# sd-james/gym-treasure-game

Hardware: AMD Instinct MI355X
Metric: env-steps/sec (whole node) at 1M batched envs, 1/2/4/8 MI355X; bit-exact vs CPU (higher is better)
Workload: dtype int32+f64

## Files before the change

gym-treasure-game_amd/csrc/tg_core.h:

```cpp
#pragma once
#include <hip/hip_runtime.h>
#include <stdint.h>

#define TG_HD __host__ __device__ __forceinline__

namespace tg {

constexpr int S = 48;
constexpr int INCR = S / 10;
constexpr int HALFW = S / 4;
constexpr int MT_N = 624, MT_M = 397;
constexpr int TICK_CAP = 1 << 14;
constexpr uint32_t TICK_DRAWS = 8;
constexpr uint32_t MAX_TICK_DRAWS = 48;
constexpr int PAD = 2;

enum : uint32_t { B_OPEN = 1, B_LADDER = 2, B_WALL = 4, B_DOOR = 8, B_DOOROBJ = 16  };
enum : int { P_NOP = 0, P_UP, P_DOWN, P_LEFT, P_RIGHT, P_JUMP, P_INTERACT };
enum : int { O_GO_LEFT = 0, O_GO_RIGHT, O_UP_LADDER, O_DOWN_LADDER, O_INTERACT, O_DOWN_LEFT,
             O_DOWN_RIGHT, O_JUMP_LEFT, O_JUMP_RIGHT, O_COUNT };

constexpr uint32_t F_JT = 0x1Fu;
constexpr uint32_t F_FACING = 1u << 5;
constexpr int F_OBJ = 6;
// ... 133 lines not shown
};
__host__ __device__ inline __attribute__((noinline)) WordPair mt_pair_ool(const uint32_t* mt, uint32_t p) {
  WordPair r;
  mt_pair(mt, p, r.w0, r.w1);
  return r;
}
TG_HD uint32_t mt_half(uint32_t pos) { return pos >= (uint32_t)MT_HALF ? (uint32_t)MT_HALF : 0u; }

constexpr int MT_CODES = MT_WORDS / 2;
constexpr uint32_t CODE_POS = 3u;
constexpr uint32_t CODE_NEG_SHIFT = 2;
constexpr uint32_t CODE_JUMP = 1u << 4;
constexpr uint32_t CODE_FLIP = 1u << 5;
TG_HD uint32_t draw_code(double r) {
  const uint32_t pos = (uint32_t)((int)rint(2.0 + 2.0 * r) - 2);
  const uint32_t neg = (uint32_t)((int)rint(-4.0 + 2.0 * r) + 4);
  return pos | (neg << CODE_NEG_SHIFT) | (r > 0.25 ? CODE_JUMP : 0u) | (r <= 0.8 ? CODE_FLIP : 0u);
}
constexpr uint32_t CODE_SLOW = 0xFFu;
TG_HD uint32_t code_of_top27(uint32_t a) {
  constexpr uint32_t Q1 = 1u << 25, Q3 = 3u << 25, F8 = 107374182u;
  if (a - (Q1 - 1u) < 3u || a - (Q3 - 1u) < 3u || a - (F8 - 1u) < 3u) return CODE_SLOW;
  constexpr uint32_t LOW = CODE_FLIP;
  constexpr uint32_t MID = 1u | (1u << CODE_NEG_SHIFT) | CODE_JUMP | CODE_FLIP;
  constexpr uint32_t HIGH = 2u | (2u << CODE_NEG_SHIFT) | CODE_JUMP;
  return a < Q1 ? LOW : a < Q3 ? MID : a < F8 ? (HIGH | CODE_FLIP) : HIGH;
}
TG_HD uint32_t draw_code_words(uint32_t w0, uint32_t w1) {
  const uint32_t c = code_of_top27(mt_temper(w0) >> 5);
  return c != CODE_SLOW ? c : draw_code(mt_double(w0, w1));
}
constexpr uint32_t TOP27_F8 = 107374182u;
constexpr uint32_t TOP27_LUT = CODE_FLIP |
                               ((1u | (1u << CODE_NEG_SHIFT) | CODE_JUMP | CODE_FLIP) << 8) |
                               ((1u | (1u << CODE_NEG_SHIFT) | CODE_JUMP | CODE_FLIP) << 16) |
                               ((2u | (2u << CODE_NEG_SHIFT) | CODE_JUMP | CODE_FLIP) << 24);
static_assert(TOP27_F8 >= (3u << 25), "only the top class splits at 0.8");
TG_HD bool top27_slow(uint32_t a) {
  return (((a + 1u) & 0x1FFFFFFu) < 3u) | (a - (TOP27_F8 - 1u) < 3u);
}
TG_HD uint32_t top27_code(uint32_t a) {
  const uint32_t c = (TOP27_LUT >> ((a >> 22) & 0x18u)) & 0xFFu;
  return a >= TOP27_F8 ? c ^ CODE_FLIP : c;
}
TG_HD int code_step(uint32_t c, bool neg) {
  return neg ? (int)((c >> CODE_NEG_SHIFT) & 3u) - 4 : (int)(c & CODE_POS) + 2;
}
TG_HD void gen_codes(const uint32_t* words, uint8_t* c) {
  for (int k = 0; k < MT_N / 2; ++k) c[k] = (uint8_t)draw_code(mt_double(words[2 * k], words[2 * k + 1]));
}
struct GenOps {
  TG_HD void twist(const uint32_t* src, uint32_t* dst) const { twist_gen(src, dst); }
  TG_HD void codes(const uint32_t* w, uint8_t* c) const { gen_codes(w, c); }
};
template <class Ops = GenOps>
TG_HD void twist_half(uint32_t* mt, uint32_t h, uint8_t* mc = nullptr, bool seeded = false,
                      const Ops& op = Ops()) {
  const uint32_t g0 = h / (uint32_t)MT_N;
  uint32_t* const s = mt + mt_store_off(g0);
  uint32_t* const s3 = s + 3 * MT_N;
  if (!seeded) op.twist(mt + mt_store_off((g0 + (uint32_t)MT_HALF_GENS + 6u) % (2u * MT_HALF_GENS)), s3);
  uint8_t* const c = mc ? mc + h / 2 : nullptr;
  const int last = c ? MT_HALF_GENS : MT_HALF_GENS - 1;
  for (int g = 0; g < last; ++g) {
    const int to = (g + 1) >> 1 < 3 ? (g + 1) >> 1 : 3;
    const uint32_t* const from = g == 0 ? s3 : (g & 1) ? s + (g >> 1) * MT_N : s + to * MT_N;
    op.twist(from, s + to * MT_N);
    if (c) op.codes(s + to * MT_N, c + g * (MT_N / 2));
  }
  if (c) {
    op.twist(s + 2 * MT_N, s3);
    op.twist(s3, s3);
  }
}

template <int DIR, class R>
TG_HD int walk_ticks(R& rng, int& x, int lim, int cap) {
  int t = 0;
  while ((DIR > 0 ? x <= lim : x >= lim) && rng.has(TICK_DRAWS) && t < cap) {
    x += code_step(rng.code(), DIR < 0);
    ++t;
  }
  return t;
}

struct Rng {
  uint32_t* mt;
  uint32_t pos;
  uint32_t draws;
  bool crossed;
  bool entered;
  uint8_t* mc;

  TG_HD Rng(uint32_t* m, uint32_t state, uint8_t* c = nullptr)
      : mt(m), pos(state & MT_POS_MASK), draws(0u), crossed((state & MT_STALE) != 0u),
        entered(false), mc(c) {}

  TG_HD double random() {
    uint32_t w0, w1;
    mt_pair_branchy(mt, pos, w0, w1);
    pos += 2;
    if (pos == (uint32_t)MT_WORDS) pos = 0u;
    if (pos == 0u || pos == (uint32_t)MT_HALF) {
      if (crossed) twist_half(mt, pos, mc);
      crossed = entered = true;
    }
    ++draws;
    return mt_double(w0, w1);
  }
  TG_HD double uniform(double a, double b) { return a + (b - a) * random(); }
  TG_HD uint32_t code() { return draw_code(random()); }
  TG_HD void reserve(uint32_t) {}
  TG_HD bool has(uint32_t) const { return true; }
  TG_HD bool overrun() const { return false; }
  TG_HD void phase(int) {}
  template <int DIR>
  TG_HD int walk(int& x, int lim, int cap) { return walk_ticks<DIR>(*this, x, lim, cap); }
  TG_HD uint32_t finish() const { return pos | (crossed ? MT_STALE : 0u); }
  TG_HD uint32_t finish_queued() const { return pos | (entered ? MT_STALE : 0u); }
};
TG_HD uint32_t refill_after(uint32_t* mt, uint32_t state, uint8_t* mc = nullptr) {
  const uint32_t pos = state & MT_POS_MASK;
  if (state & MT_STALE) twist_half(mt, (uint32_t)MT_HALF - mt_half(pos), mc);
  return pos;
}

TG_HD void seed_mt(uint32_t* mt, const uint32_t* genrand19650218, uint64_t seed) {
  const uint32_t key0 = (uint32_t)seed, key1 = (uint32_t)(seed >> 32);
  const uint32_t klen = key1 ? 2u : 1u;
  uint32_t prev = genrand19650218[0];
  uint32_t m0 = prev;
  uint32_t j = 0;
  uint32_t i = 1;
  for (int k = 0; k < MT_N; ++k) {
    const uint32_t cur = (i == 1 && k == MT_N - 1) ? mt[1] : genrand19650218[i];
    const uint32_t key = (j == 0) ? key0 : key1;
    const uint32_t v = (cur ^ ((prev ^ (prev >> 30)) * 1664525u)) + key + j;
    mt[i] = v;
    prev = v;
    ++i;
    ++j;
    if (i >= (uint32_t)MT_N) { m0 = mt[MT_N - 1]; prev = m0; i = 1; }
    if (j >= klen) j = 0;
  }
  mt[0] = m0;
  for (int k = 0; k < MT_N - 1; ++k) {
    const uint32_t cur = mt[i];
    const uint32_t v = (cur ^ ((prev ^ (prev >> 30)) * 1566083941u)) - i;
    mt[i] = v;
    prev = v;
    ++i;
    if (i >= (uint32_t)MT_N) { mt[0] = mt[MT_N - 1]; prev = mt[0]; i = 1; }
  }
  mt[0] = 0x80000000u;
}
constexpr uint32_t MT_SEED_OFF = 3 * MT_N;
TG_HD void init_mt(uint32_t* mt, const uint32_t* genrand19650218, uint64_t seed,
                   uint8_t* mc = nullptr) {
  seed_mt(mt + MT_SEED_OFF, genrand19650218, seed);
  twist_half(mt, 0u, mc, true);
  twist_half(mt, (uint32_t)MT_HALF, mc);
}

struct AirCells {
  uint32_t oA, oB, bA, bB;
  int bx, by1;
// ... 703 lines not shown
    if (!pr.lad(DIR, y) || pr.fall(dc, y)) break;
    int end;
    if (DIR < 0) {
      end = max(max(floordiv(y - INCR, S) * S + INCR, floordiv(y, S) * S),
                max(floordiv(y + S - INCR, S) * S - (S - INCR), floordiv(y + S + 2, S) * S - (S + 2)));
      end = max(end, bound);
    } else {
      end = min(min(floordiv(y, S) * S + S - 1, floordiv(y + S / 2, S) * S + S - 1 - S / 2),
                min(floordiv(y + S + INCR - 1, S) * S + S - 1 - (S + INCR - 1),
                    floordiv(y + S + 2, S) * S + S - 1 - (S + 2)));
      end = min(end, bound);
    }
    lim = end;
    y = end + DIR;
  }
  return lim;
}

template <int K, class R>
TG_HD int air_tick(const Level& L, const uint32_t* trig, const Map& m, Env& e, Opt& o, R& rng,
                   AirCells& ac) {
  constexpr int DIR = (K == O_JUMP_LEFT || K == O_DOWN_LEFT) ? -1 : 1;
  constexpr bool JUMP = K == O_JUMP_LEFT || K == O_JUMP_RIGHT;
  const uint32_t dc = Map::dc_of(e.f);
  if (!ac.holds(dc, e.px, e.py)) {
    ac = m.air_cells(dc, e.px, e.py);
    if (!ac.holds(dc, e.px, e.py)) {
      const int prim = policy<K>(L, m, e, o);
      return tick<prims_of(K), R>(L, trig, m, e, prim, rng);
    }
  }
  const AirProbe ap(ac, e.px, e.py);
  const bool cf0 = ap.can_fall();
  const bool fwd = ap.side(DIR);
  int mv = 0;
  if (close_x(e, o.tx)) {
    if (!cf0) o.done = true;
  } else {
    mv = (JUMP && !cf0 && !fwd) ? -DIR : DIR;
  }
  int xd = 0, yd = 0;
  if (mv != 0 && (mv == DIR ? fwd : ap.side(-DIR))) {
    xd = code_step(rng.code(), mv < 0);
    e.f = mv > 0 ? (e.f | F_FACING) : (e.f & ~F_FACING);
  }
  const uint32_t jt = e.f & F_JT;
  if (jt > 0) {
    if (ap.up_clear()) yd = -INCR;
    e.f = (e.f & ~F_JT) | (jt - 1);
  } else if (cf0) {
    yd = INCR;
  }
  e.px += xd;
  if (yd > 0) yd = ap.fall(e.px, yd);
  e.py += yd;
  pickups(L, e);
  return -1;
}

template <int DIR, class R>
TG_HD int ladder_tick(const Level& L, const Map& m, const LadMasks& lm, Env& e, Opt& o, R& rng) {
  int yd = 0;
  if (DIR < 0 ? lm.can_go_up(m, e.py) : lm.can_go_down(m, e.py)) yd = code_step(rng.code(), DIR < 0);
  else o.done = true;
  const uint32_t jt = e.f & F_JT;
  if (jt > 0) {
    if (lm.up_clear(m, e.py)) yd = -INCR;
    e.f = (e.f & ~F_JT) | (jt - 1);
  } else if (lm.can_fall(m, e.py)) {
    yd = INCR;
  }
  if (yd > 0) yd = lm.fall_dist(m, e.py, yd);
  e.py += yd;
  pickups(L, e);
  return -1;
}

template <int DIR, class R, class P, class Full>
TG_HD void ladder_loop(const Level& L, const Map& m, Env& e, Opt& o, R& rng, StepResult& r,
                       const P& pr, Full full) {
  int lim = DIR > 0 ? -0x40000000 : 0x40000000;
  do {
    rng.phase(0);
    bool capped = false;
    while ((DIR > 0 ? e.py <= lim : e.py >= lim) && rng.has(TICK_DRAWS)) {
      e.py += code_step(rng.code(), DIR < 0);
      r.reward += -1;
      if (DIR > 0 ? e.py > lim : e.py < lim) pickups(L, e);
      if (++r.ticks >= TICK_CAP) {
        e.f |= E_TICKCAP;
        capped = true;
        lim = DIR > 0 ? -0x40000000 : 0x40000000;
      }
    }
    if (capped) break;
    rng.phase(1);
    rng.reserve(TICK_DRAWS);
    rng.phase(2);
    r.reward += full();
    if (!o.done) lim = ladder_plain_limit<DIR>(m, e, pr);
    rng.phase(3);
    if (++r.ticks >= TICK_CAP) {
      e.f |= E_TICKCAP;
      break;
    }
  } while (!o.done);
}

template <int K, class R>
TG_HD void run_option_k(const Level& L, const uint32_t* trig, const Map& m, Env& e, R& rng,
                        StepResult& r) {
  r.ran = 1;
  Opt o{0, false, false};
  if constexpr (K == O_GO_LEFT || K == O_GO_RIGHT) {
    constexpr int DIR = K == O_GO_LEFT ? -1 : 1;
    int lim = DIR > 0 ? -0x40000000 : 0x40000000;
    do {
      rng.phase(0);
      if (const int t = rng.template walk<DIR>(e.px, lim, TICK_CAP - r.ticks)) {
        e.f = DIR > 0 ? (e.f | F_FACING) : (e.f & ~F_FACING);
        r.reward -= t;
        r.ticks += t;
        if (DIR > 0 ? e.px > lim : e.px < lim) pickups(L, e);
        if (r.ticks >= TICK_CAP) {
          e.f |= E_TICKCAP;
          break;
        }
      }
      rng.phase(1);
      rng.reserve(TICK_DRAWS);
      rng.phase(2);
      const int prim = policy<K>(L, m, e, o);
      r.reward += tick<prims_of(K), R>(L, trig, m, e, prim, rng);
      if (!o.done) lim = go_plain_limit<DIR>(m, e, o.tx);
      rng.phase(3);
      if (++r.ticks >= TICK_CAP) {
        e.f |= E_TICKCAP;
        break;
      }
    } while (!o.done);
    return;
  }
  if constexpr (K == O_UP_LADDER || K == O_DOWN_LADDER) {
    constexpr int DIR = K == O_UP_LADDER ? -1 : 1;
    if (m.mk) {
      const LadMasks lm(m, Map::dc_of(e.f), e.px);
      ladder_loop<DIR>(L, m, e, o, rng, r, LadProbeMk{m, lm},
                       [&]() { return ladder_tick<DIR>(L, m, lm, e, o, rng); });
      return;
    }
    ladder_loop<DIR>(L, m, e, o, rng, r, LadProbe{m, e}, [&]() {
      const int prim = policy<K>(L, m, e, o);
      return tick<prims_of(K), R>(L, trig, m, e, prim, rng);
    });
    return;
  }
  if constexpr (K == O_JUMP_LEFT || K == O_JUMP_RIGHT || K == O_DOWN_LEFT || K == O_DOWN_RIGHT) {
    AirCells ac{0u, 0u, 0u, 0u, -0x40000000, 0, 0u};
    do {
      rng.phase(0);
      rng.phase(1);
      rng.reserve(TICK_DRAWS);
      rng.phase(2);
      if (o.init) {
        r.reward += air_tick<K>(L, trig, m, e, o, rng, ac);
      } else {
        const int prim = policy<K>(L, m, e, o);
        r.reward += tick<prims_of(K), R>(L, trig, m, e, prim, rng);
      }
      rng.phase(3);
      if (++r.ticks >= TICK_CAP) {
        e.f |= E_TICKCAP;
        break;
      }
    } while (!o.done);
    return;
  }
  do {
    rng.reserve(K == O_INTERACT ? L.interact_draws : TICK_DRAWS);
    const int prim = policy<K>(L, m, e, o);
    r.reward += tick<prims_of(K), R>(L, trig, m, e, prim, rng);
    if (++r.ticks >= TICK_CAP) {
      e.f |= E_TICKCAP;
      break;
    }
  } while (!o.done);
}
template <class R>
TG_HD void run_option(const Level& L, const uint32_t* trig, const Map& m, Env& e, int k,
                      R& rng, StepResult& r) {
  switch (k) {
    case O_GO_LEFT: run_option_k<O_GO_LEFT>(L, trig, m, e, rng, r); break;
    case O_GO_RIGHT: run_option_k<O_GO_RIGHT>(L, trig, m, e, rng, r); break;
    case O_UP_LADDER: run_option_k<O_UP_LADDER>(L, trig, m, e, rng, r); break;
    case O_DOWN_LADDER: run_option_k<O_DOWN_LADDER>(L, trig, m, e, rng, r); break;
    case O_INTERACT: run_option_k<O_INTERACT>(L, trig, m, e, rng, r); break;
    case O_DOWN_LEFT: run_option_k<O_DOWN_LEFT>(L, trig, m, e, rng, r); break;
    case O_DOWN_RIGHT: run_option_k<O_DOWN_RIGHT>(L, trig, m, e, rng, r); break;
    case O_JUMP_LEFT: run_option_k<O_JUMP_LEFT>(L, trig, m, e, rng, r); break;
    default: run_option_k<O_JUMP_RIGHT>(L, trig, m, e, rng, r); break;
  }
}
TG_HD int option_index(int a) {
  if (a < -O_COUNT || a >= O_COUNT) return -1;
  return a < 0 ? a + O_COUNT : a;
}
template <class R>
TG_HD StepResult env_step(const Level& L, const uint32_t* trig, const Map& m, Env& e, int a,
                          R& rng) {
  StepResult r{0, 0, 0, 0};
  const int k = option_index(a);
  if (k < 0) e.f |= E_ACTION;
  else if (can_run(L, m, e, k)) run_option(L, trig, m, e, k, rng, r);
  r.done = is_done(e);
  return r;
}

}
```

gym-treasure-game_amd/csrc/tg_dev.h:

```cpp
#pragma once
#include <hip/hip_runtime.h>

#include "../../include/tg_amd.h"
#include "tg_core.h"
#include "tg_level.h"
#include "tg_batch.h"
#include "tg_twist.h"

using namespace tg;

namespace {

constexpr int BLOCK = 256;
#ifndef TG_RUN_BLOCK
#define TG_RUN_BLOCK 256
#endif
constexpr int RUN_BLOCK = TG_RUN_BLOCK;
static_assert(RUN_BLOCK % 64 == 0 && BLOCK % RUN_BLOCK == 0, "whole waves, whole k_classify blocks");
constexpr int PRIO_SLOW = 3;

__device__ __forceinline__ void unpack_st4(const uint4 s, Env& e) {
  e.px = (int)(int16_t)(s.x & 0xFFFFu);
  e.py = (int)(int16_t)(s.x >> 16);
  e.f = s.y;
// ... 119 lines not shown
__device__ __noinline__ WordPair mt_pair_ool_sc1(const uint32_t* mt, uint32_t p) {
  WordPair r;
  mt_pair(mt, p, r.w0, r.w1, Sc1Ld());
  return r;
}

template <bool FLOW = false>
struct RngCodesT {
  static constexpr uint32_t NONE = 0xFFFFFFFFu;
  uint32_t* mt;
  uint8_t* mc;
  lds_u8* cell;
  uint32_t m0;
  uint32_t pos;
  uint32_t n;
  uint32_t rd;
  uint32_t left;
  uint32_t nxc;
  uint32_t stale;
  uint32_t tag;
  uint32_t draws;
  uint32_t regens;
  bool primed, loaded, entered;

  __device__ __forceinline__ RngCodesT(uint32_t* m, uint8_t* c, uint32_t state, lds_u8* wave_win)
      : mt(m), mc(c), cell(wave_win + (threadIdx.x & 63) * WIN_UNIT),
        m0(__builtin_amdgcn_readfirstlane((uint32_t)(uintptr_t)wave_win)),
        pos(state & MT_POS_MASK), n(0u), rd(0u), left(0u), nxc(0u),
        stale((state & MT_STALE) ? (uint32_t)MT_HALF - mt_half(state & MT_POS_MASK) : NONE),
        tag(state & (MT_STALE | MT_LISTED)),
        draws(0u), regens(0u), primed(false), loaded(false), entered(false) {}

  __device__ __forceinline__ void sync() {
    const uint32_t d = pos >> 1, e = d + n;
    if (e / (MT_HALF / 2) != d / (MT_HALF / 2)) {
      const uint32_t left_half = mt_half(pos), entered_half = (uint32_t)MT_HALF - left_half;
      if (stale == entered_half) {
        if (FLOW) regen_half_flow(mt, mc, entered_half);
        else regen_half(mt, mc, entered_half);
        ++regens;
      }
      stale = left_half;
      entered = true;
    }
    pos = 2u * (e >= (uint32_t)MT_CODES ? e - (uint32_t)MT_CODES : e);
    n = 0u;
  }
  __device__ __forceinline__ void fill() {
    const uint32_t d = pos >> 1, c0 = d / (uint32_t)WIN_UNIT;
    if (stale != NONE) {
      const uint32_t w0 = pos, w1 = pos + 2u * ((uint32_t)WIN_DRAWS - d % (uint32_t)WIN_UNIT);
      if ((w0 < stale + (uint32_t)MT_HALF && stale < w1) ||
          (w1 > (uint32_t)MT_WORDS && stale < w1 - (uint32_t)MT_WORDS)) {
        if (FLOW) regen_half_flow(mt, mc, stale);
        else regen_half(mt, mc, stale);
        ++regens;
        stale = NONE;
      }
    }
#pragma unroll
    for (int j = 0; j < WIN_SLOTS; ++j) {
      const uint32_t c = c0 + j < CODE_UNITS ? c0 + j : c0 + j - CODE_UNITS;
      glds_unit<FLOW>(m0 + j * WIN_SLOT_BYTES, mc + c * (uint32_t)WIN_UNIT);
    }
    rd = d % (uint32_t)WIN_UNIT;
    left = (uint32_t)WIN_DRAWS - rd;
    loaded = false;
  }
  __device__ __forceinline__ uint32_t read() const {
    const uint32_t r = rd < (uint32_t)WIN_DRAWS ? rd : 0u;
    return cell[(r / WIN_UNIT) * WIN_SLOT_BYTES + r % WIN_UNIT];
  }
  __device__ __forceinline__ void prime() {
    fill();
    primed = true;
  }
  __device__ __forceinline__ void reserve(uint32_t k) {
    if (!primed) prime();
    if (left < k) {
      asm volatile("s_waitcnt lgkmcnt(0)" ::: "memory");
      sync();
      fill();
    }
    if (!loaded) {
      asm volatile("s_waitcnt vmcnt(0)" ::: "memory");
      nxc = read();
      loaded = true;
    }
  }
  __device__ __forceinline__ bool has(uint32_t k) const { return left >= k; }
  __device__ __forceinline__ uint32_t dword(uint32_t d) const {
    return *reinterpret_cast<const lds_u32*>(cell + (4u * d / WIN_UNIT) * WIN_SLOT_BYTES +
                                             (4u * d) % WIN_UNIT);
  }
  template <int DIR>
  __device__ __forceinline__ int walk(int& x, const int lim, const int cap) {
    int taken = 0;
    if (!((DIR > 0 ? x <= lim : x >= lim) && left >= TICK_DRAWS && cap > 0)) return 0;
    uint32_t w = dword(rd >> 2);
    while (true) {
      const uint32_t wn = dword((rd >> 2) + 1u);
      const int k = (int)(rd & 3u);
      int moved = 0;
      bool act = true;
#pragma unroll
      for (int i = 0; i < 4; ++i) {
        const int st = code_step((w >> (8 * i)) & 0xFFu, DIR < 0);
        act = act && (i >= k ? ((DIR > 0 ? x <= lim : x >= lim) &&
                                left - (uint32_t)moved >= TICK_DRAWS && taken + moved < cap)
                             : true);
        if (i >= k && act) {
          x += st;
          ++moved;
        }
      }
      taken += moved;
      rd += (uint32_t)moved;
      left -= (uint32_t)moved;
      n += (uint32_t)moved;
      draws += (uint32_t)moved;
      if (moved < 4 - k) break;
      if (!((DIR > 0 ? x <= lim : x >= lim) && left >= TICK_DRAWS && taken < cap)) break;
      w = wn;
    }
    nxc = read();
    return taken;
  }
#ifdef TG_DIAG_STAMPS
  unsigned long long ph[4] = {0, 0, 0, 0}, last = 0;
  uint32_t rounds = 0;
  __device__ __forceinline__ void phase(int k) {
    const unsigned long long now = __builtin_amdgcn_s_memtime();
    if (last) ph[k] += now - last;
    last = now;
    rounds += k == 0;
  }
#else
  __device__ __forceinline__ void phase(int) {}
#endif
  __device__ __forceinline__ bool overrun() const { return left > (uint32_t)WIN_DRAWS; }
  __device__ __forceinline__ uint32_t code() {
    const uint32_t c = nxc;
    ++n;
    ++draws;
    ++rd;
    --left;
    nxc = read();
    return c;
  }
  __device__ __forceinline__ double random() {
    uint32_t p = (pos >> 1) + n;
    p = 2u * (p >= (uint32_t)MT_CODES ? p - (uint32_t)MT_CODES : p);
    (void)code();
    const WordPair w = FLOW ? mt_pair_ool_sc1(mt, p) : mt_pair_ool(mt, p);
    return mt_double(w.w0, w.w1);
  }
  __device__ __forceinline__ double uniform(double a, double b) { return a + (b - a) * random(); }
  __device__ __forceinline__ uint32_t finish() {
    if (primed) asm volatile("s_waitcnt vmcnt(0) lgkmcnt(0)" ::: "memory");
    sync();
    primed = loaded = false;
    return pos | (stale == NONE ? 0u : entered ? MT_STALE : tag);
  }
};

using RngCodes = RngCodesT<false>;

__device__ __forceinline__ uint64_t readlane64(uint64_t v, int lane) {
  const uint32_t lo = __builtin_amdgcn_readlane((uint32_t)v, lane);
  const uint32_t hi = __builtin_amdgcn_readlane((uint32_t)(v >> 32), lane);
  return ((uint64_t)hi << 32) | lo;
}
__device__ __forceinline__ void wave_refill(unsigned long long need, uint32_t* env_mt, uint8_t* env_mc,
                                            uint32_t state, lds_u32* scratch) {
  const uint32_t pos = state & MT_POS_MASK;
  const uint32_t dst = (uint32_t)MT_HALF - mt_half(pos);
  const uint64_t src_l = (uint64_t)(uintptr_t)(env_mt + regen_src_off(dst));
  const uint64_t w_l = (uint64_t)(uintptr_t)env_mt;
  const uint64_t c_l = (uint64_t)(uintptr_t)env_mc;
  const int g0_l = (int)(dst / (uint32_t)MT_N);
  while (need) {
    const int L = __ffsll((long long)need) - 1;
    need &= need - 1;
    wave_twist_gens((const glb_u32*)(uintptr_t)readlane64(src_l, L),
                    (glb_u32*)(uintptr_t)readlane64(w_l, L), (uint8_t*)(uintptr_t)readlane64(c_l, L),
                    __builtin_amdgcn_readlane(g0_l, L), MT_HALF_GENS, true, scratch);
  }
}

__device__ __forceinline__ int wave_sum(int v) {
#pragma unroll
  for (int o = 32; o > 0; o >>= 1) v += __shfl_xor(v, o, 64);
  return v;
}

enum { ST_STEPS, ST_VALID, ST_TICKS, ST_DRAWS, ST_EPISODES, ST_EP_OVERFLOW, ST_REGENS, ST_WTICKS,
       ST_COUNT };

__device__ __forceinline__ int wave_max(int v) {
#pragma unroll
  for (int o = 32; o > 0; o >>= 1) v = max(v, __shfl_xor(v, o, 64));
  return v;
}

constexpr int KST_SLOTS = 64;
constexpr int KST_STRIDE = 16;
__device__ __forceinline__ unsigned long long kst_begin(const unsigned long long* ks) {
  return ks ? __builtin_amdgcn_s_memrealtime() : 0ull;
}
__device__ __forceinline__ void kst_end(unsigned long long* ks, unsigned long long t0) {
  if (ks && (threadIdx.x & 63) == 0) {
    unsigned long long* const s = ks + KST_STRIDE * (blockIdx.x % KST_SLOTS);
    atomicMin(s, t0);
    atomicMax(s + 1, (unsigned long long)__builtin_amdgcn_s_memrealtime());
  }
}
struct StepIO {
  int32_t* __restrict__ actions;
  double* __restrict__ obs;
  int32_t* __restrict__ reward;
  uint8_t* __restrict__ valid;
  uint8_t* __restrict__ done;
  double* __restrict__ final_obs;
  int policy;
  uint64_t a0;
  int64_t t;
  uint32_t tstep;
};

__device__ __forceinline__ uint64_t sm64(uint64_t x) {
  x += 0x9E3779B97F4A7C15ull;
  x = (x ^ (x >> 30)) * 0xBF58476D1CE4E5B9ull;
  x = (x ^ (x >> 27)) * 0x94D049BB133111EBull;
  return x ^ (x >> 31);
}
__device__ __forceinline__ int policy_action(const Level& L, const Map& m, const Env& e,
                                             int policy, uint64_t a0, int64_t g, int64_t t) {
  const uint64_t h = sm64(sm64(a0 ^ sm64((uint64_t)g)) ^ (uint64_t)t);
  int a = (int)(h % 9ull);
  if (policy == TG_POLICY_MASKED) {
    const uint32_t mk = available_mask(L, m, e);
    const int c = __popc(mk);
// ... 69 lines not shown
  const int v[5] = {steps, valid, ticks, draws, episodes};
#pragma unroll
  for (int c = 0; c < 5; ++c)
    if (v[c]) atomicAdd(&slot[c], (unsigned long long)v[c]);
  if (regens) atomicAdd(&slot[ST_REGENS], (unsigned long long)regens);
  if (wave_ticks && ticks) atomicAdd(&slot[ST_WTICKS], (unsigned long long)ticks);
}

__device__ __forceinline__ Level level_div(const Level& L) {
  Level d = L;
  d.obs_q = nullptr;
  return d;
}
template <bool AUTORESET, bool FINAL, bool VALID = true, class R>
__device__ __forceinline__ void finish_step(const Level& L, Env& e, R& rng, int64_t i,
                                            const StepResult& r, int2& ep, const StepIO& io,
                                            double* keep = nullptr) {
  if (rng.overrun()) e.f |= E_WINDOW;
  double o[9];
  observe(L, e, o);
  io.reward[i] = r.reward;
  if (VALID) io.valid[i] = (uint8_t)r.ran;
  io.done[i] = (uint8_t)r.done;
  ep.x += r.reward;
  if (FINAL) store_obs(io.final_obs, i, o);
  if (AUTORESET && r.done) {
    reset_env(L, e, rng);
    observe(L, e, o);
  }
  if (keep) {
#pragma unroll
    for (int k = 0; k < 9; ++k) keep[k] = o[k];
  } else {
    store_obs(io.obs, i, o);
  }
}

__device__ __forceinline__ void store_obs_wave(double* __restrict__ out, int64_t wave_first,
                                               unsigned long long mask, const double o[9],
                                               double* __restrict__ stage) {
  const int lane = threadIdx.x & 63;
#pragma unroll
  for (int k = 0; k < 9; ++k) stage[lane * 9 + k] = o[k];
  __builtin_amdgcn_fence(__ATOMIC_RELEASE, "wavefront");
  __builtin_amdgcn_wave_barrier();
  __builtin_amdgcn_fence(__ATOMIC_ACQUIRE, "wavefront");
  double* const dst = out + wave_first * 9;
#pragma unroll
  for (int j = 0; j < 9; ++j) {
    const int w = j * 64 + lane;
    if ((mask >> (w / 9)) & 1ull) __builtin_nontemporal_store(stage[w], dst + w);
  }
}

constexpr int POL_IMMEDIATE = -2;
template <bool AUTORESET, bool FINAL, int POL, bool ONE = false>
__device__ __forceinline__ StepResult step_env(const Soa& S, int64_t n, const Level& L,
                                         const uint32_t* trig, const Map& m, lds_u8* wscr,
                                         int64_t i, const StepIO& io, const EpQueue& q,
                                         int64_t g0, unsigned long long* __restrict__ stats,
                                         uint32_t* __restrict__ err_or) {
  const bool live = i < n;
  StepResult r{0, 0, 0, 0};
  uint32_t draws = 0;
  int lregen = 0;
  Env e;
  e.mti = 0u;
  int2 ep = make_int2(0, 0), ep_in = ep;
  if (live) {
    unpack(S.st4[i], S.ang[i], e);
    ep = S.ep[i];
    ep_in = ep;
    RngCodes rng(S.mt + i * MT_STORE, S.mc + i * MT_CODES, e.mti, wscr);
    int act;
    if constexpr (POL >= 0) {
      act = policy_action(L, m, e, POL, io.a0, g0 + i, io.t);
      if (io.actions) io.actions[i] = act;
    } else if constexpr (POL == POL_IMMEDIATE) {
      act = (int)(int64_t)io.a0;
    } else {
      act = io.actions[i];
    }
    r = env_step(L, trig, m, e, act, rng);
    finish_step<AUTORESET, FINAL>(level_div(L), e, rng, i, r, ep, io);
    e.mti = rng.finish();
    draws = rng.draws;
    lregen = (int)rng.regens;
    if (e.f & E_MASK) atomicOr(err_or, e.f & E_MASK);
  }
  const unsigned long long need = __ballot(live && (e.mti & MT_STALE));
  wave_refill(need, S.mt + (live ? i : 0) * MT_STORE,
              S.mc + (live ? i : 0) * MT_CODES, e.mti,
              (lds_u32*)wscr);
  e.mti &= ~(MT_STALE | MT_LISTED);
  if (AUTORESET) record_episodes(live && r.done, g0 + i, ep, io.tstep, q, stats, blockIdx.x);
  if (live) {
    S.st4[i] = pack(e);
    S.ang[i] = make_double2(e.ang0, e.ang1);
    if (ep.x != ep_in.x || ep.y != ep_in.y) S.ep[i] = ep;
  }
  if constexpr (ONE)
    lane0_stats(stats, live ? 1 : 0, r.ran, r.ticks, (int)draws, AUTORESET ? (live && r.done) : 0,
                __popcll(need) + lregen, true);
  else
    wave_stats(stats, live ? 1 : 0, r.ran, r.ticks, (int)draws, AUTORESET ? (live && r.done) : 0,
               __popcll(need) + wave_sum(lregen), true);
  return r;
}

constexpr int SHARDS = 8;
#ifndef TG_WSHARDS
#define TG_WSHARDS 8
#endif
constexpr int WSHARDS = TG_WSHARDS;
constexpr int L_RESET = O_COUNT;
constexpr int NLIST = O_COUNT + 1;
constexpr int kOrderH[NLIST] = {O_JUMP_LEFT, O_JUMP_RIGHT, O_GO_LEFT,     O_GO_RIGHT,
                                O_DOWN_LEFT, O_DOWN_RIGHT, O_UP_LADDER,   O_DOWN_LADDER,
                                O_INTERACT,  L_RESET};
struct RunPos {
  int of[NLIST];
};
constexpr RunPos make_runpos() {
  RunPos r{};
  for (int j = 0; j < NLIST; ++j) r.of[kOrderH[j]] = j;
  return r;
}
constexpr RunPos kRunPos = make_runpos();
constexpr int NSEG = NLIST * WSHARDS;
static_assert(NSEG <= 2 * RUN_BLOCK, "k_run's prefix: two segments per thread");
constexpr int NCTR = NSEG;
constexpr int CTR_STRIDE = 32;
struct Work {
  int32_t* __restrict__ lists;
  uint4* __restrict__ wst4;
  double2* __restrict__ wang;
  int2* __restrict__ wep;
  int32_t* __restrict__ ctr;
  int32_t* __restrict__ ctr_next;
  uint32_t* __restrict__ refill;
  int32_t* __restrict__ rcnt;
  int64_t rcap;
  int64_t shard_cap;
};
constexpr int REGEN_STEPS = 16;
constexpr int RCTR_LIST = 8;
constexpr int RCTR_N = 16;
}

namespace tg {
const void* flow_kernel(bool ar, int pol);
}
```

gym-treasure-game_amd/csrc/tg_kernels.h:

```cpp
#pragma once
#include "tg_dev.h"
#include "tg_flow.h"
#include "tg_policy_mlp.h"

namespace {

__global__ void k_kst_init(unsigned long long* ks, int64_t slots) {
  const int64_t i = (int64_t)blockIdx.x * blockDim.x + threadIdx.x;
  if (i < slots) {
    ks[KST_STRIDE * i] = ~0ull;
    ks[KST_STRIDE * i + 1] = 0ull;
  }
}

__global__ __launch_bounds__(BLOCK) void k_create(Soa S, int64_t n, uint64_t seed0,
                                                   const uint32_t* __restrict__ genrand) {
  const int64_t i = (int64_t)blockIdx.x * BLOCK + threadIdx.x;
  if (i >= n) return;
  seed_mt(S.mt + i * MT_STORE + MT_SEED_OFF, genrand, seed0 + (uint64_t)i);
  Env e{};
  e.mti = 0u;
  S.st4[i] = pack(e);
  S.ang[i] = make_double2(0.0, 0.0);
  S.ep[i] = make_int2(0, 0);
// ... 226 lines not shown
    const int c1 = s0 + 1 < NSEG ? w.ctr[(s0 + 1) * CTR_STRIDE] : 0;
    int v = c0 + c1;
#pragma unroll
    for (int o = 1; o < 64; o <<= 1) {
      const int y = __shfl_up(v, o, 64);
      if (ln >= o) v += y;
    }
    if (ln == 63) wtot[threadIdx.x >> 6] = v;
    __syncthreads();
    for (int wv = 0; wv < (int)(threadIdx.x >> 6); ++wv) v += wtot[wv];
    const int excl = v - c0 - c1;
    if (s0 < NSEG) pre[s0] = excl;
    if (s0 + 1 < NSEG) pre[s0 + 1] = excl + c0;
    if (threadIdx.x == RUN_BLOCK - 1) pre[NSEG] = v;
  }
  __syncthreads();
  if ((int)(blockIdx.x * RUN_BLOCK) >= pre[NSEG] + NLIST * 63) {
    kst_end(ks, kt0);
    return;
  }
  if (threadIdx.x == 0) {
    int acc = 0;
    for (int j = 0; j < NLIST; ++j) {
      const int sb = j * WSHARDS, se = sb + WSHARDS;
      ostart[j] = acc;
      oraw[j] = pre[sb];
      acc += (pre[se] - pre[sb] + 63) & ~63;
    }
    ostart[NLIST] = acc;
    oraw[NLIST] = pre[NSEG];
  }
  RUN_LEVEL_IN_LDS();
  const int total = ostart[NLIST];
  const int base = (blockIdx.x * RUN_BLOCK + threadIdx.x) & ~63;
  int oj = 0;
  while (oj + 1 < NLIST && ostart[oj + 1] <= base) ++oj;
  oj = __builtin_amdgcn_readfirstlane(oj);
  const int k = kOrder[oj];
  const int qraw = oraw[oj] + base + (threadIdx.x & 63) - ostart[oj];
  const bool live = base < total && qraw < oraw[oj + 1];
  int seg = oj * WSHARDS;
  if (live) {
    int hi = seg + WSHARDS;
    while (hi - seg > 1) {
      const int mid = (seg + hi) >> 1;
      if (pre[mid] <= qraw) seg = mid; else hi = mid;
    }
  }
  const int idx = qraw - pre[seg];
  int64_t i = 0;
  StepResult r{0, 0, 0, 0};
  Env e;
  e.mti = 0u;
  int2 ep = make_int2(0, 0);
  uint32_t draws = 0;
  int regens = 0;
  int lregen = 0;
  lds_u8* const wscr = (lds_u8*)win + (threadIdx.x >> 6) * WIN_WAVE_BYTES;
  unsigned long long t0 = 0, t1 = 0, t2 = 0, t3 = 0;
  TG_STAMP(t0);
#ifdef TG_DIAG_STAMPS
  const unsigned long long rt0 = __builtin_amdgcn_s_memrealtime();
#endif
  (void)t0; (void)t1; (void)t2; (void)t3;
#ifdef TG_DIAG_STAMPS
  unsigned long long ph1 = 0, ph2 = 0, ph3 = 0;
  uint32_t prounds = 0;
#endif
  if (live) {
    const int64_t at = (int64_t)seg * w.shard_cap + idx;
    i = w.lists[at];
    unpack(w.wst4[at], w.wang[at], e);
    ep = w.wep[at];
    RngCodes rng(S.mt + i * MT_STORE, S.mc + i * MT_CODES, e.mti, wscr);
    rng.prime();
    TG_STAMP(t1);
    if (k != O_GO_LEFT && k != O_GO_RIGHT && k != O_INTERACT) __builtin_amdgcn_s_setprio(PRIO_SLOW);
    if (k != L_RESET) run_option(L, trig, m, e, k, rng, r);
    TG_STAMP(t2);
#ifdef TG_DIAG_STAMPS
    ph1 = rng.ph[1], ph2 = rng.ph[2], ph3 = rng.ph[3], prounds = rng.rounds;
#endif
    r.done = is_done(e);
    finish_step<AUTORESET, FINAL, false>(level_div(L), e, rng, i, r, ep, io);
    e.mti = rng.finish();
    draws = rng.draws;
    lregen = (int)rng.regens;
    if (e.f & E_MASK) atomicOr(err_or, e.f & E_MASK);
  }
  if (AUTORESET)
    record_episodes(live && r.done, g0 + i, ep, io.tstep, q, stats, (int64_t)blockIdx.x / (BLOCK / RUN_BLOCK));
  if (live) {
    S.st4[i] = pack(e);
    S.ang[i] = make_double2(e.ang0, e.ang1);
    S.ep[i] = ep;
  }
  __builtin_amdgcn_s_setprio(0);
  wave_stats(stats, 0, 0, r.ticks, (int)draws, AUTORESET ? (live && r.done) : 0,
             regens + (__ballot(lregen != 0) ? wave_sum(lregen) : 0), true,
             (int64_t)blockIdx.x / (BLOCK / RUN_BLOCK));
  kst_end(ks, kt0);
#ifdef TG_DIAG_STAMPS
  TG_STAMP(t3);
  {
    int mx = r.ticks;
    for (int o = 32; o > 0; o >>= 1) mx = max(mx, __shfl_xor(mx, o, 64));
    const int sum = wave_sum(r.ticks);
    const unsigned long long bl = __ballot(live);
    const int src = bl ? __ffsll((long long)bl) - 1 : 0;
    const unsigned long long a1 = __shfl(t1, src, 64);
    const unsigned long long a2 = __shfl(t2, src, 64);
    const int wv = (blockIdx.x * RUN_BLOCK + threadIdx.x) >> 6;
    const unsigned long long rt3 = __builtin_amdgcn_s_memrealtime();
    int lmax = src;
    unsigned long long best = 0;
    for (int l = 0; l < 64; ++l) {
      const unsigned long long tl = __shfl(ph1 + ph2 + ph3, l, 64);
      if (((bl >> l) & 1ull) && tl > best) best = tl, lmax = l;
    }
    const unsigned long long p1 = __shfl(ph1, lmax, 64), p2 = __shfl(ph2, lmax, 64),
                             p3 = __shfl(ph3, lmax, 64);
    const uint32_t pr = __shfl(prounds, lmax, 64);
    if ((threadIdx.x & 63) == 0 && wv < NSTAMP_WAVES) {
      unsigned long long* const g = g_stamps + (size_t)wv * NSTAMP;
      g[0] = bl ? a1 - t0 : 0;
      g[1] = bl ? a2 - a1 : 0;
      g[2] = bl ? t3 - a2 : t3 - t0;
      g[3] = bl ? (unsigned long long)mx | ((unsigned long long)sum << 32) | ((unsigned long long)k << 56)
                : 1ull | (15ull << 56);
      g[4] = rt0;
      g[5] = rt3;
      g[6] = p1;
      g[7] = p2;
      g[8] = p3;
      g[9] = pr;
      g[10] = (unsigned long long)regens;
    }
  }
#endif
}

#ifndef TG_REGEN_NT
#define TG_REGEN_NT 0
#endif
constexpr bool REGEN_NT = TG_REGEN_NT != 0;
__global__ __launch_bounds__(BLOCK) void k_regen(Soa S, const uint32_t* __restrict__ refill,
                                                 int64_t rcap, int32_t* __restrict__ ctr,
                                                 int32_t* __restrict__ ctr_next,
                                                 unsigned long long* __restrict__ stats,
                                                 int nstat, unsigned long long* __restrict__ ks) {
  const unsigned long long kt0 = kst_begin(ks);
  __shared__ __attribute__((aligned(16))) uint32_t scratch[BLOCK / 64][MT_N];
  lds_u32* const scr = (lds_u32*)scratch[threadIdx.x >> 6];
  const int lane = threadIdx.x & 63;
  const int xcd = (int)(blockIdx.x & 7u);
  const int64_t cnt = ctr[(RCTR_LIST + xcd) * CTR_STRIDE];
  if (blockIdx.x == 0 && threadIdx.x < RCTR_N) ctr_next[threadIdx.x * CTR_STRIDE] = 0;
  int32_t* const q = ctr + xcd * CTR_STRIDE;
  const uint32_t* const list = refill + xcd * rcap;
  uint32_t* const st_w = reinterpret_cast<uint32_t*>(S.st4);
  auto src_of = [&](uint32_t env, uint32_t s) {
    const uint32_t dst = (uint32_t)MT_HALF - mt_half(s & MT_POS_MASK);
    return (const glb_u32*)(S.mt + (int64_t)env * MT_STORE + regen_src_off(dst));
  };
  const int wx = (int)(blockIdx.x >> 3) * (BLOCK / 64) + (int)(threadIdx.x >> 6);
  const int64_t nwx = (int64_t)((gridDim.x - (unsigned)xcd + 7u) >> 3) * (BLOCK / 64);
// ... 191 lines not shown
```

Measured before the change: 9.855 billion.

## Batch RNG walk ticks via packed prefix sums and route ladder walks through window

The per-draw walk loop becomes a hop scheme. Four step codes packed in one dword are summed with a multiply-based prefix, so whole groups of four ticks advance in one comparison. The ladder plain-walk loop now uses the window's batched walk instead of drawing one code at a time, and the air-option loop is peeled so the first policy tick runs separately from the air_tick loop. The code also adds a drain/land split so the pending code load is waited on before finish_step rather than in finish, and defines unused ring-buffer helpers. These changes aim to cut per-tick instruction count and branching, at the risk of subtle bit-exactness issues in the hop-distance boundary logic.

```diff
diff --git a/gym-treasure-game_amd/csrc/tg_core.h b/gym-treasure-game_amd/csrc/tg_core.h
--- a/gym-treasure-game_amd/csrc/tg_core.h
+++ b/gym-treasure-game_amd/csrc/tg_core.h
@@ -239,6 +239,101 @@
     ++t;
   }
   return t;
+}
+
+TG_HD uint32_t hop_prefix(uint32_t w, bool neg) {
+  return ((neg ? w >> CODE_NEG_SHIFT : w) & 0x03030303u) * 0x01010101u;
+}
+TG_HD int hop_dist(uint32_t p, int j, bool neg) {
+  const int s = j ? (int)((p >> (8 * (j - 1))) & 0xFFu) : 0;
+  return neg ? 4 * j - s : 2 * j + s;
+}
+template <int DIR>
+TG_HD bool hop_ticks(uint32_t w, int m, int& x, int lim, uint32_t left, int taken, int cap) {
+  const uint32_t p = hop_prefix(w, DIR < 0);
+  const int d = DIR > 0 ? lim - x : x - lim;
+  if (!(hop_dist(p, m - 1, DIR < 0) <= d && left >= TICK_DRAWS + (uint32_t)(m - 1) &&
+        taken + m - 1 < cap))
+    return false;
+  x += DIR * hop_dist(p, m, DIR < 0);
+  return true;
+}
+template <int DIR, class W>
+TG_HD int walk_hops(W& win, int& x, int lim, int cap) {
+  int taken = 0;
+  bool whole = true;
+  if (const int k = (int)(win.rd & 3u)) {
+    const int m = 4 - k;
+    whole = (DIR > 0 ? x <= lim : x >= lim) && win.left >= TICK_DRAWS &&
+            hop_ticks<DIR>(win.dword(win.rd >> 2) >> (8 * k), m, x, lim, win.left, 0, cap);
+    if (whole) taken = m, win.rd += (uint32_t)m, win.left -= (uint32_t)m;
+  }
+  if (whole) {
+    int d = DIR > 0 ? lim - x : x - lim;
+    const int room = cap - 3 - taken;
+    uint32_t i = win.rd >> 2, left = win.left;
+    const uint32_t left0 = left;
+    const bool in = d >= 0;
+    uint32_t w = in && left >= TICK_DRAWS + 3u ? win.dword(i) : 0u;
+    while (in && left >= TICK_DRAWS + 3u && (int)(left0 - left) < room) {
+      const uint32_t wn = win.dword(i + 1u);
+      const uint32_t p = hop_prefix(w, DIR < 0);
+      if (hop_dist(p, 3, DIR < 0) > d) break;
+      d -= hop_dist(p, 4, DIR < 0);
+      ++i;
+      left -= 4u;
+      w = wn;
+    }
+    x = DIR > 0 ? lim - d : lim + d;
+    taken += (int)(left0 - left);
+    win.rd = 4u * i;
+    win.left = left;
+  }
+  if ((DIR > 0 ? x <= lim : x >= lim) && win.left >= TICK_DRAWS && taken < cap) {
+    const uint32_t w = win.dword(win.rd >> 2);
+    const int k = (int)(win.rd & 3u);
+    int moved = 0;
+    bool act = true;
+#pragma unroll
+    for (int i = 0; i < 4; ++i) {
+      const int st = code_step((w >> (8 * i)) & 0xFFu, DIR < 0);
+      act = act && (i >= k ? ((DIR > 0 ? x <= lim : x >= lim) &&
+                              win.left - (uint32_t)moved >= TICK_DRAWS && taken + moved < cap)
+                           : true);
+      if (i >= k && act) {
+        x += st;
+        ++moved;
+      }
+    }
+    taken += moved;
+    win.rd += (uint32_t)moved;
+    win.left -= (uint32_t)moved;
+  }
+  return taken;
+}
+
+constexpr uint32_t RING_UNIT = 16, RING_SLOTS = 4, RING_DRAWS = RING_UNIT * RING_SLOTS;
+constexpr uint32_t RING_UNITS = MT_CODES / RING_UNIT;
+static_assert((MT_CODES / 2) % RING_UNIT == 0, "a half of the ring is whole units");
+TG_HD uint32_t ring_slot(uint32_t rd) { return (rd / RING_UNIT) % RING_SLOTS; }
+TG_HD uint32_t ring_free(uint32_t rd, uint32_t staged) {
+  return RING_SLOTS - (rd % RING_UNIT + staged) / RING_UNIT;
+}
+TG_HD uint32_t ring_order(uint32_t rd, uint32_t staged, uint32_t j) {
+  return (j - (rd + staged) / RING_UNIT) % RING_SLOTS;
+}
+TG_HD uint32_t ring_unit(uint32_t u, uint32_t k) {
+  return u + k >= RING_UNITS ? u + k - RING_UNITS : u + k;
+}
+TG_HD uint32_t ring_next_unit(uint32_t cur, uint32_t staged) {
+  return ((cur + staged) / RING_UNIT) % RING_UNITS;
+}
+TG_HD uint32_t ring_plan(uint32_t pos, uint32_t rd, uint32_t staged, uint32_t cur) {
+  const uint32_t f = ring_free(rd, staged);
+  if (!f) return 0u;
+  const uint32_t u = ring_next_unit(cur, staged), per_half = RING_UNITS / 2u;
+  const uint32_t h = pos >= (uint32_t)MT_HALF ? 1u : 0u;
+  return (u / per_half == h && (u + f - 1u) / per_half == h) ? f : 0u;
 }
 
 struct Rng {
@@ -1108,18 +1203,15 @@
   int lim = DIR > 0 ? -0x40000000 : 0x40000000;
   do {
     rng.phase(0);
-    bool capped = false;
-    while ((DIR > 0 ? e.py <= lim : e.py >= lim) && rng.has(TICK_DRAWS)) {
-      e.py += code_step(rng.code(), DIR < 0);
-      r.reward += -1;
+    if (const int t = rng.template walk<DIR>(e.py, lim, TICK_CAP - r.ticks)) {
+      r.reward -= t;
+      r.ticks += t;
       if (DIR > 0 ? e.py > lim : e.py < lim) pickups(L, e);
-      if (++r.ticks >= TICK_CAP) {
+      if (r.ticks >= TICK_CAP) {
         e.f |= E_TICKCAP;
-        capped = true;
-        lim = DIR > 0 ? -0x40000000 : 0x40000000;
+        break;
       }
     }
-    if (capped) break;
     rng.phase(1);
     rng.reserve(TICK_DRAWS);
     rng.phase(2);
@@ -1183,23 +1275,31 @@
   }
   if constexpr (K == O_JUMP_LEFT || K == O_JUMP_RIGHT || K == O_DOWN_LEFT || K == O_DOWN_RIGHT) {
     AirCells ac{0u, 0u, 0u, 0u, -0x40000000, 0, 0u};
-    do {
+    {
       rng.phase(0);
       rng.phase(1);
       rng.reserve(TICK_DRAWS);
       rng.phase(2);
-      if (o.init) {
-        r.reward += air_tick<K>(L, trig, m, e, o, rng, ac);
-      } else {
-        const int prim = policy<K>(L, m, e, o);
-        r.reward += tick<prims_of(K), R>(L, trig, m, e, prim, rng);
+      const int prim = policy<K>(L, m, e, o);
+      r.reward += tick<prims_of(K), R>(L, trig, m, e, prim, rng);
+      rng.phase(3);
+      if (++r.ticks >= TICK_CAP) {
+        e.f |= E_TICKCAP;
+        return;
       }
+    }
+    while (!o.done) {
+      rng.phase(0);
+      rng.phase(1);
+      rng.reserve(TICK_DRAWS);
+      rng.phase(2);
+      r.reward += air_tick<K>(L, trig, m, e, o, rng, ac);
       rng.phase(3);
       if (++r.ticks >= TICK_CAP) {
         e.f |= E_TICKCAP;
         break;
       }
-    } while (!o.done);
+    }
     return;
   }
   do {
diff --git a/gym-treasure-game_amd/csrc/tg_dev.h b/gym-treasure-game_amd/csrc/tg_dev.h
--- a/gym-treasure-game_amd/csrc/tg_dev.h
+++ b/gym-treasure-game_amd/csrc/tg_dev.h
@@ -225,6 +225,9 @@
       sync();
       fill();
     }
+    land();
+  }
+  __device__ __forceinline__ void land() {
     if (!loaded) {
       asm volatile("s_waitcnt vmcnt(0)" ::: "memory");
       nxc = read();
@@ -238,34 +241,9 @@
   }
   template <int DIR>
   __device__ __forceinline__ int walk(int& x, const int lim, const int cap) {
-    int taken = 0;
-    if (!((DIR > 0 ? x <= lim : x >= lim) && left >= TICK_DRAWS && cap > 0)) return 0;
-    uint32_t w = dword(rd >> 2);
-    while (true) {
-      const uint32_t wn = dword((rd >> 2) + 1u);
-      const int k = (int)(rd & 3u);
-      int moved = 0;
-      bool act = true;
-#pragma unroll
-      for (int i = 0; i < 4; ++i) {
-        const int st = code_step((w >> (8 * i)) & 0xFFu, DIR < 0);
-        act = act && (i >= k ? ((DIR > 0 ? x <= lim : x >= lim) &&
-                                left - (uint32_t)moved >= TICK_DRAWS && taken + moved < cap)
-                             : true);
-        if (i >= k && act) {
-          x += st;
-          ++moved;
-        }
-      }
-      taken += moved;
-      rd += (uint32_t)moved;
-      left -= (uint32_t)moved;
-      n += (uint32_t)moved;
-      draws += (uint32_t)moved;
-      if (moved < 4 - k) break;
-      if (!((DIR > 0 ? x <= lim : x >= lim) && left >= TICK_DRAWS && taken < cap)) break;
-      w = wn;
-    }
+    const int taken = walk_hops<DIR>(*this, x, lim, cap);
+    n += (uint32_t)taken;
+    draws += (uint32_t)taken;
     nxc = read();
     return taken;
   }
@@ -299,8 +277,15 @@
     return mt_double(w.w0, w.w1);
   }
   __device__ __forceinline__ double uniform(double a, double b) { return a + (b - a) * random(); }
+  __device__ __forceinline__ void drain() {
+    if (primed) land();
+  }
   __device__ __forceinline__ uint32_t finish() {
-    if (primed) asm volatile("s_waitcnt vmcnt(0) lgkmcnt(0)" ::: "memory");
+    if constexpr (FLOW) {
+      if (primed) asm volatile("s_waitcnt vmcnt(0) lgkmcnt(0)" ::: "memory");
+    } else {
+      drain();
+    }
     sync();
     primed = loaded = false;
     return pos | (stale == NONE ? 0u : entered ? MT_STALE : tag);
@@ -536,6 +521,7 @@
       act = io.actions[i];
     }
     r = env_step(L, trig, m, e, act, rng);
+    rng.drain();
     finish_step<AUTORESET, FINAL>(level_div(L), e, rng, i, r, ep, io);
     e.mti = rng.finish();
     draws = rng.draws;
diff --git a/gym-treasure-game_amd/csrc/tg_kernels.h b/gym-treasure-game_amd/csrc/tg_kernels.h
--- a/gym-treasure-game_amd/csrc/tg_kernels.h
+++ b/gym-treasure-game_amd/csrc/tg_kernels.h
@@ -332,6 +332,7 @@
     ph1 = rng.ph[1], ph2 = rng.ph[2], ph3 = rng.ph[3], prounds = rng.rounds;
 #endif
     r.done = is_done(e);
+    rng.drain();
     finish_step<AUTORESET, FINAL, false>(level_div(L), e, rng, i, r, ep, io);
     e.mti = rng.finish();
     draws = rng.draws;
```

After: 10.12 billion, median of 6. +2.7%, better.
